# folkol/query-engines

Hardware: AMD Instinct MI355X
Metric: rows/sec filter+project+group-by over 1B-row Arrow batch; % HBM roofline (higher is better)
Workload: dtype int64; 1 GPU; C4: SELECT k, SUM(a+b), COUNT(*), MIN(a), MAX(b) WHERE a > 2^19 GROUP BY k; rows_per_gpu=1000000000, groups=1024, columns=k, a, b int64 (Arrow, no nulls), parallelism=hash-sharded partial aggregate x1

## Files before the change

query-engines_amd/csrc/qe_hashagg.hip:

```cpp
#include <map>
#include <memory>
#include <mutex>

#include "qe_internal.hpp"

namespace qe {

constexpr int HA_THREADS = 512;

__device__ __forceinline__ qi64* lds_keys(char* smem) { return (qi64*)smem; }

__device__ __forceinline__ void lds_init(const Plan& P, char* smem) {
  const int SS = (1 << P.lds_log2) + 2;
  qi64* keys = lds_keys(smem);
  qu32* cst = (qu32*)(smem + P.off_cstar);
  for (int s = threadIdx.x; s < SS; s += blockDim.x) {
    keys[s] = EMPTY_KEY;
    cst[s] = 0;
  }
#pragma unroll
  for (int j = 0; j < QE_MAX_AGGS; ++j) {
    if (j >= P.naggs) break;
    const DAgg& a = P.aggs[j];
    if (a.acc != ACC_NONE) {
      qi64* acc = (qi64*)(smem + P.off_acc[j]);
      const qi64 id = acc_identity(a.acc);
      for (int s = threadIdx.x; s < SS; s += blockDim.x) acc[s] = id;
    }
    if (a.track_nn) {
      qu32* nn = (qu32*)(smem + P.off_nn[j]);
      for (int s = threadIdx.x; s < SS; s += blockDim.x) nn[s] = 0;
    }
    if (acc_has_idx(a.acc)) {
      qu64* ix = (qu64*)(smem + P.off_idx[j]);
      const qu64 id = idx_identity(a.acc);
      for (int s = threadIdx.x; s < 4 * SS; s += blockDim.x) ix[s] = id;
    }
  }
}

__device__ __forceinline__ int lds_find(const Plan& P, char* smem, qi64 key, bool knull) {
  const int S = 1 << P.lds_log2;
  if (knull) return S;
  if (key == EMPTY_KEY) return S + 1;
  return lds_probe(lds_keys(smem), P.lds_log2, key, lds_hash((qu64)key) >> (32 - P.lds_log2));
}

__device__ __forceinline__ void lds_accum_value(const Plan& P, char* smem, int j, int s, qi64 x, qu64 row) {
  const DAgg& a = P.aggs[j];
  qi64* acc = (qi64*)(smem + P.off_acc[j]);
  switch (a.acc) {
    case ACC_SUM_I: atomicAdd((unsigned long long*)&acc[s], (unsigned long long)x); break;
// ... 816 lines not shown
    }
  }
}

__global__ void k_nn_materialize(DTable t, qi32 mask) {
  const qu64 SS = t.cap + 2;
  for (qu64 s = blockIdx.x * (qu64)blockDim.x + threadIdx.x; s < SS; s += (qu64)gridDim.x * blockDim.x)
    for (int j = 0; j < QE_MAX_AGGS; ++j)
      if ((mask >> j) & 1) t.nn[j][s] = t.cstar[s];
}

__device__ __forceinline__ bool gslot_occupied(const DTable& t, qu64 s) {
  return s < t.cap ? t.keys[s] != EMPTY_KEY : t.cstar[s] > 0;
}

__device__ __forceinline__ void wg_newg_begin(qu32* newg) {
  if (threadIdx.x == 0) *newg = 0;
  __syncthreads();
}
__device__ __forceinline__ void wg_newg_end(qu32* newg, qu64* ctl) {
  __syncthreads();
  if (threadIdx.x == 0 && *newg) atomicAdd((unsigned long long*)&ctl[0], (unsigned long long)*newg);
}

__global__ void k_rehash(DTable src, DTable dst, AggMeta m) {
  __shared__ qu32 newg;
  wg_newg_begin(&newg);
  const qu64 SS = src.cap + 2;
  for (qu64 s = blockIdx.x * (qu64)blockDim.x + threadIdx.x; s < SS; s += (qu64)gridDim.x * blockDim.x) {
    if (!gslot_occupied(src, s)) continue;
    const bool knull = s == src.cap;
    const qi64 key = knull ? 0 : (s == src.cap + 1 ? EMPTY_KEY : src.keys[s]);
    qu64 d;
    if (!gtable_find_wg(dst, key, knull, d, &newg)) {
      atomicAdd((unsigned long long*)&dst.ctl[3], 1ull);
      continue;
    }
    gadd_cstar(dst, d, src.cstar[s]);
    for (int j = 0; j < m.naggs; ++j) {
      DAgg a{};
      a.fn = m.fn[j];
      a.acc = m.acc[j];
      qu64 i[4] = {~0ull, ~0ull, ~0ull, ~0ull};
      if (acc_has_idx(a.acc))
        for (int k = 0; k < 4; ++k) i[k] = src.idx[j][k * SS + s];
      gcombine(dst, a.acc, j, d, src.acc[j][s], slot_nn(src, m, j, s), i[0], i[1], i[2], i[3]);
      if (a.acc == ACC_SUM_X && (i[3] & FX_EXT))
        fxe_add_words<true>(dst.ext[j] + d * FXE_WORDS, 0, src.ext[j] + s * FXE_WORDS, FXE_WORDS);
    }
  }
  wg_newg_end(&newg, dst.ctl);
}

__device__ void import_record(const qu8* __restrict__ rec, DTable& dst, const AggMeta& m, qu32* newg) {
  const qi64 key = ((const qi64*)rec)[0];
  const bool knull = ((const qu64*)rec)[1] & 1;
  const qu64 c = ((const qu64*)rec)[2];
  qu64 d;
  if (!gtable_find_wg(dst, key, knull, d, newg)) {
    atomicAdd((unsigned long long*)&dst.ctl[3], 1ull);
    return;
  }
  gadd_cstar(dst, d, c);
  int off = 24;
  for (int j = 0; j < m.naggs; ++j) {
    DAgg a{};
    a.fn = m.fn[j];
    a.acc = m.acc[j];
    const qu64* f = (const qu64*)(rec + off);
    if (a.fn != QE_AGG_COUNT_STAR) {
      if (acc_has_idx(a.acc)) gcombine(dst, a.acc, j, d, (qi64)f[0], f[1], f[2], f[3], f[4], f[5]);
      else gcombine(dst, a.acc, j, d, (qi64)f[0], f[1], ~0ull, ~0ull, ~0ull, ~0ull);
    }
    off += agg_rec_bytes(a.acc);
  }
}

__global__ void k_import(const qu8* __restrict__ recs, qi64 nrec, qi32 rec_bytes, DTable dst, AggMeta m) {
  __shared__ qu32 newg;
  wg_newg_begin(&newg);
  for (qi64 r = blockIdx.x * (qi64)blockDim.x + threadIdx.x; r < nrec; r += (qi64)gridDim.x * blockDim.x)
    import_record(recs + r * rec_bytes, dst, m, &newg);
  wg_newg_end(&newg, dst.ctl);
}

__global__ void k_import_slots(const qu8* __restrict__ slots, qi32 nslots, qi64 slot_records, qi32 rec_bytes,
                               DTable dst, AggMeta m) {
  __shared__ qu32 newg;
  __shared__ qi32 s_ok;
  const qu64 slot_bytes = QE_SLOT_HEADER + (qu64)slot_records * rec_bytes;
  if (threadIdx.x < 64) {
    qu64 mx = 0, tot = 0;
    for (int i = threadIdx.x; i < nslots; i += 64) {
      const qu64* hd = (const qu64*)(slots + (qu64)i * slot_bytes);
      mx = hd[1] > mx ? hd[1] : mx;
      tot += hd[0] < (qu64)slot_records ? hd[0] : (qu64)slot_records;
    }
    for (int off = 32; off > 0; off >>= 1) {
      const qu64 o = __shfl_xor(mx, off);
      mx = o > mx ? o : mx;
      tot += __shfl_xor(tot, off);
    }
    if (threadIdx.x == 0) {
      s_ok = mx <= (qu64)slot_records;
      if (blockIdx.x == 0) {
        dst.ctl[4] = mx;
        dst.ctl[5] = tot;
      }
    }
  }
  wg_newg_begin(&newg);
  if (s_ok) {
    const qi64 total = (qi64)nslots * slot_records;
    for (qi64 r = blockIdx.x * (qi64)blockDim.x + threadIdx.x; r < total; r += (qi64)gridDim.x * blockDim.x) {
      const qi64 sl = r / slot_records, i = r - sl * slot_records;
      const qu8* base = slots + (qu64)sl * slot_bytes;
      if ((qu64)i >= ((const qu64*)base)[0]) continue;
      import_record(base + QE_SLOT_HEADER + (qu64)i * rec_bytes, dst, m, &newg);
    }
  }
  wg_newg_end(&newg, dst.ctl);
// ... 100 lines not shown
    const bool has = s < SS && gslot_occupied(t, s);
    const bool knull = s == t.cap;
    const qi64 key = !has ? 0 : knull ? 0 : (s == t.cap + 1 ? EMPTY_KEY : t.keys[s]);
    const qu32 p = has ? partition_of(key, knull, nparts) : 0;
    const qu64 pos = wave_cursor(cursor, has, p);
    if (has) write_record(dst + pos * (qu64)rec_bytes, t, m, s, key, knull);
    if (m.any_x) {
      const bool ext = has && slot_has_ext(t, m, s);
      const qu64 pe = wave_cursor(cursor, ext, p, FXE_CHUNKS);
      if (ext)
        for (int c = 0; c < FXE_CHUNKS; ++c) write_chunk_record(dst + (pe + c) * (qu64)rec_bytes, t, m, s, key, knull, c);
    }
  }
}

__global__ void k_export_slots(DTable t, AggMeta m, qi32 nparts, qi32 rec_bytes, qi64 slot_records,
                               unsigned long long* cursor, qu8* __restrict__ dst) {
  const qu64 SS = t.cap + 2;
  const qu64 slot_bytes = QE_SLOT_HEADER + (qu64)slot_records * rec_bytes;
  const qu64 stride = (qu64)gridDim.x * blockDim.x;
  for (qu64 s0 = blockIdx.x * (qu64)blockDim.x; s0 < SS; s0 += stride) {
    const qu64 s = s0 + threadIdx.x;
    const bool has = s < SS && gslot_occupied(t, s);
    const bool knull = s == t.cap;
    const qi64 key = !has ? 0 : knull ? 0 : (s == t.cap + 1 ? EMPTY_KEY : t.keys[s]);
    const qu32 p = has ? partition_of(key, knull, nparts) : 0;
    const qu64 pos = wave_cursor(cursor, has, p);
    qu8* base = dst + p * slot_bytes + QE_SLOT_HEADER;
    if (has && pos < (qu64)slot_records) write_record(base + pos * (qu64)rec_bytes, t, m, s, key, knull);
    if (m.any_x) {
      const bool ext = has && slot_has_ext(t, m, s);
      const qu64 pe = wave_cursor(cursor, ext, p, FXE_CHUNKS);
      if (ext)
        for (int c = 0; c < FXE_CHUNKS; ++c)
          if (pe + c < (qu64)slot_records) write_chunk_record(base + (pe + c) * (qu64)rec_bytes, t, m, s, key, knull, c);
    }
  }
}

__global__ void k_slot_headers(const unsigned long long* __restrict__ cursor, qi32 nparts, qu64 slot_bytes,
                               qu8* __restrict__ dst, const qu64* __restrict__ guard) {
  qu64 mx = 0;
  for (int p = threadIdx.x; p < nparts; p += blockDim.x) mx = cursor[p] > mx ? cursor[p] : mx;
  for (int off = 32; off > 0; off >>= 1) {
    const qu64 o = __shfl_xor(mx, off);
    mx = o > mx ? o : mx;
  }
  if (guard && (guard[1] | guard[2] | guard[3])) mx = 1ull << 62;
  for (int p = threadIdx.x; p < nparts; p += blockDim.x) {
    qu64* hd = (qu64*)(dst + (qu64)p * slot_bytes);
    hd[0] = cursor[p];
    hd[1] = mx;
    for (int w = 2; w < QE_SLOT_HEADER / 8; ++w) hd[w] = 0;
  }
}

__global__ void k_occ_count(DTable t, qi64* __restrict__ tile_counts, qi32 tile_slots) {
  __shared__ qi64 part[4];
  const qu64 SS = t.cap + 2;
  const qu64 s0 = (qu64)blockIdx.x * tile_slots;
  qi64 c = 0;
  for (int i = threadIdx.x; i < tile_slots; i += blockDim.x) {
    const qu64 s = s0 + i;
    if (s < SS && gslot_occupied(t, s)) ++c;
  }
  for (int off = 32; off > 0; off >>= 1) c += __shfl_xor(c, off);
  if ((threadIdx.x & 63) == 0) part[threadIdx.x >> 6] = c;
  __syncthreads();
  if (threadIdx.x == 0) tile_counts[blockIdx.x] = part[0] + part[1] + part[2] + part[3];
}

struct OutCols {
  qe_column keys[QE_MAX_KEYS];
  qe_column aggs[QE_MAX_AGGS];
};

__device__ __forceinline__ void set_bit(qu8* bm, qi64 i, bool v) {
  if (v) atomicOr((qu32*)bm + (i >> 5), 1u << (i & 31));
}

__device__ __forceinline__ void store_typed(void* p, qi32 type, qi64 i, qi64 x) {
  switch (type) {
    case QE_TYPE_INT64:
    case QE_TYPE_FLOAT64: ((qi64*)p)[i] = x; break;
    case QE_TYPE_INT32:
    case QE_TYPE_DATE32: ((qi32*)p)[i] = (qi32)x; break;
    default: ((qu8*)p)[i] = (qu8)x;
  }
}

constexpr int FS_WORDS = 512;
__device__ __forceinline__ void put_bit(qu8* gbm, qu32* lbits, int col, qi64 o, bool v) {
  if (!v) return;
  if (lbits) atomicOr(lbits + col * FS_WORDS + (o >> 5), 1u << (o & 31));
  else set_bit(gbm, o, true);
}

__device__ __forceinline__ double fx_sum(const DTable& t, int j, qu64 s, qi64 acc) {
  const qu64 SS = t.cap + 2;
  const qu64* ix = t.idx[j];
  return fx_result((qu64)acc, ix[s], ix[SS + s], ix[2 * SS + s], ix[3 * SS + s], t.ext[j] + s * FXE_WORDS);
}

__device__ __forceinline__ void finalize_slot(const DTable& t, const AggMeta& m, const KeyMeta& km,
                                              const OutCols& out, qu64 s, qi64 o, qu32* lbits = nullptr) {
  const qu64 SS = t.cap + 2;
// ... 25 lines not shown
      case QE_AGG_AVG:
        if (m.acc[j] == ACC_SUM_X)
          val = f64_bits(fx_sum(t, j, s, acc) / (double)nn);
        else
          val = f64_bits(bits_f64(acc) / (double)nn);
        break;
      default:
        if (m.acc[j] == ACC_SUM_X) {
          val = f64_bits(fx_sum(t, j, s, acc));
        } else if (acc_is_f64mm(m.acc[j])) {
          const qu64 i0 = t.idx[j][s], i1 = t.idx[j][SS + s];
          const qu64 i2 = t.idx[j][2 * SS + s], i3 = t.idx[j][3 * SS + s];
          if (i1 != ~0ull && i1 == i0) {
            val = 0x7FF8000000000000ll;
          } else {
            const double d = okey_f64(acc);
            val = d == 0.0 ? f64_bits(i2 < i3 ? -0.0 : 0.0) : f64_bits(d);
          }
        } else {
          val = acc;
        }
    }
    ((qi64*)out.aggs[j].values)[o] = valid ? val : 0;
    if (out.aggs[j].validity) put_bit(out.aggs[j].validity, lbits, QE_MAX_KEYS + j, o, valid);
  }
}

__global__ void k_finalize(DTable t, AggMeta m, KeyMeta km, const qi64* __restrict__ tile_offsets,
                           qi32 tile_slots, OutCols out) {
  __shared__ int wtot[4];
  const qu64 SS = t.cap + 2;
  const int lane = threadIdx.x & 63, wid = threadIdx.x >> 6;
  const qu64 lt = lane ? (~0ull >> (64 - lane)) : 0ull;
  qi64 base = tile_offsets[blockIdx.x];
  for (int it = 0; it < tile_slots; it += blockDim.x) {
    const qu64 s = (qu64)blockIdx.x * tile_slots + it + threadIdx.x;
    const bool occ = (it + (int)threadIdx.x) < tile_slots && s < SS && gslot_occupied(t, s);
    const qu64 b = __ballot(occ);
    if (lane == 0) wtot[wid] = __popcll(b);
    __syncthreads();
    int woff = 0, btot = 0;
    for (int w = 0; w < 4; ++w) {
      woff += w < wid ? wtot[w] : 0;
      btot += wtot[w];
    }
    if (occ) finalize_slot(t, m, km, out, s, base + woff + __popcll(b & lt));
    base += btot;
    __syncthreads();
  }
}

constexpr int FS_THREADS = 1024, FS_PER = 16, FS_WAVES = FS_THREADS / 64;
static_assert(FS_THREADS * FS_PER / 2 / 32 <= FS_WORDS, "LDS bitmaps hold every group of a small table");
__global__ void __launch_bounds__(FS_THREADS) k_finalize_small(DTable t, AggMeta m, KeyMeta km, OutCols out,
                                                               qi64 groups) {
  __shared__ qi32 wcnt[FS_PER][FS_WAVES];
  __shared__ qu64 wbal[FS_PER][FS_WAVES];
  __shared__ qu32 lbits[(QE_MAX_KEYS + QE_MAX_AGGS) * FS_WORDS];
  const qu64 SS = t.cap + 2;
  const int tid = threadIdx.x, lane = tid & 63, wid = tid >> 6;
  const qu64 lt = lane ? (~0ull >> (64 - lane)) : 0ull;
  const int words = (int)((groups + 31) >> 5);
  for (int w = tid; w < (QE_MAX_KEYS + QE_MAX_AGGS) * FS_WORDS; w += FS_THREADS) lbits[w] = 0;
  qu32 occ = 0;
#pragma unroll
  for (int i = 0; i < FS_PER; ++i) {
    const qu64 s = (qu64)i * FS_THREADS + tid;
    if (s < SS && gslot_occupied(t, s)) occ |= 1u << i;
  }
#pragma unroll
  for (int i = 0; i < FS_PER; ++i) {
    const qu64 b = __ballot((occ >> i) & 1);
    if (lane == 0) {
      wbal[i][wid] = b;
      wcnt[i][wid] = __popcll(b);
    }
  }
  __syncthreads();
  static_assert(FS_PER * FS_WAVES == 4 * 64, "four (chunk, wave) counts per lane");
  if (wid == 0) {
    qi32* flat = &wcnt[0][0];
    const qi32 c0 = flat[4 * lane], c1 = flat[4 * lane + 1], c2 = flat[4 * lane + 2], c3 = flat[4 * lane + 3];
    const qi32 sum = c0 + c1 + c2 + c3;
    qi32 inc = sum;
#pragma unroll
    for (int d = 1; d < 64; d <<= 1) {
      const qi32 y = __shfl_up(inc, d);
      if (lane >= d) inc += y;
    }
    const qi32 ex = inc - sum;
    flat[4 * lane] = ex;
    flat[4 * lane + 1] = ex + c0;
    flat[4 * lane + 2] = ex + c0 + c1;
    flat[4 * lane + 3] = ex + c0 + c1 + c2;
  }
  __syncthreads();
  while (occ) {
    const int i = __ffs(occ) - 1;
    occ &= occ - 1;
    const qi64 o = wcnt[i][wid] + __popcll(wbal[i][wid] & lt);
    finalize_slot(t, m, km, out, (qu64)i * FS_THREADS + tid, o, lbits);
  }
  __syncthreads();
  for (int w = tid; w < words; w += FS_THREADS) {
    for (int k = 0; k < QE_MAX_KEYS; ++k)
      if (k < km.nkeys && out.keys[k].validity) ((qu32*)out.keys[k].validity)[w] = lbits[k * FS_WORDS + w];
// ... 5 lines not shown
}

using namespace qe;

struct qe_hashagg {
  qe_ctx* ctx = nullptr;
  int32_t nkeys = 0;
  int32_t key_types[QE_MAX_KEYS] = {};
  int32_t naggs = 0;
  qe_agg_desc aggs[QE_MAX_AGGS] = {};
  int32_t acc[QE_MAX_AGGS] = {};
  KeyMeta km{};
  int32_t rec_bytes = 0;
  int32_t nn_implicit = 0;
  int64_t row_base = 0;
  int64_t known_groups = 0;
  void* table_mem = nullptr;
  DTable t{};
  qu64* ctl = nullptr;
  int32_t lds_log2 = 0;
  int32_t lds_log2_min = 0;
  int64_t expected_groups = 0;
  int64_t create_groups = 0;
  int grid = 0;
  int64_t* part_cnt = nullptr;
  size_t part_cnt_bytes = 0;
  int64_t chunk_cap = 0;
  uint8_t* part_rec = nullptr;
  size_t part_rec_bytes = 0;
  int64_t* part_slc = nullptr;
  size_t part_slc_bytes = 0;
  bool part_wide = false;
  bool narrow_failed = false;
  bool compact_off = false;
  uint8_t* ovf = nullptr;
  uint64_t ovf_cap = 0;
  uint32_t* defer[2] = {nullptr, nullptr};
  size_t defer_words = 0;
  bool defer_dirty[2] = {false, false};
  bool ctl_rows_clean = false;
  hipEvent_t ev[2] = {nullptr, nullptr};
  double last_kernel_ms = 0.0;
  int last_launches = 0;
  int last_specialized = 0;
  uint64_t last_sig = 0;
  std::string jit_note;
  bool async = false;
  bool pending = false;
  std::unique_ptr<qe::Plan> pend_plan;
  size_t pend_lds = 0;
  int pend_out_i = 0;
  uint64_t* ctl_pin = nullptr;
  hipEvent_t ev_ctl = nullptr;
  int poisoned = 0;
  std::string poison_msg;
  qe::Keyed* keyed = nullptr;
  int32_t flags = 0;
  uint64_t version = 0;
};

namespace qe {

int hashagg_expected_groups(const qe_hashagg* h, int64_t* out) {
  QE_CHECK(h && out, QE_ERR_INVALID_ARG, "null argument");
  *out = h->create_groups;
  return QE_OK;
}

qe_ctx* hashagg_ctx(const qe_hashagg* h) { return h ? h->ctx : nullptr; }

HashaggInfo hashagg_info(const qe_hashagg* h) {
  HashaggInfo I{};
  I.ctx = h->ctx;
  I.km = h->km;
  I.rec_bytes = h->rec_bytes;
  I.naggs = h->naggs;
  I.flags = h->flags;
  for (int j = 0; j < h->naggs; ++j) I.aggs[j] = h->aggs[j];
  I.version = h->version;
  I.ctl = (uint64_t*)h->ctl;
  I.keyed = h->keyed;
  return I;
}

static AggMeta agg_meta(const qe_hashagg* h) {
  AggMeta m{};
  m.naggs = h->naggs;
  for (int j = 0; j < h->naggs; ++j) {
    m.fn[j] = h->aggs[j].fn;
    m.acc[j] = h->acc[j];
    m.any_x = m.any_x || h->acc[j] == ACC_SUM_X;
  }
  m.nn_implicit = h->nn_implicit;
  return m;
}

static int32_t all_nn_bits(const qe_hashagg* h) {
  if (!agg_knobs().nn_implicit) return 0;
  int32_t b = 0;
  for (int j = 0; j < h->naggs; ++j)
    if (h->aggs[j].fn != QE_AGG_COUNT_STAR) b |= 1 << j;
  return b;
}

static int nn_materialize(qe_hashagg* h, int32_t mask) {
  mask &= h->nn_implicit;
  if (!mask) return QE_OK;
  const int grid = (int)std::min<uint64_t>(div_up(h->t.cap + 2, 256), 4096);
  hipLaunchKernelGGL(k_nn_materialize, dim3(grid), dim3(256), 0, h->ctx->stream, h->t, (qi32)mask);
  QE_TRY(launch_check("k_nn_materialize"));
  h->nn_implicit &= ~mask;
  return QE_OK;
}

static size_t table_bytes(const qe_hashagg* h, uint64_t cap) {
  const uint64_t SS = cap + 2;
  size_t b = 16 * SS;
  for (int j = 0; j < h->naggs; ++j)
    b += (16 + (acc_has_idx(h->acc[j]) ? 32 : 0) + (h->acc[j] == ACC_SUM_X ? 8 * FXE_WORDS : 0)) * SS;
  return b;
}

static int table_alloc(qe_hashagg* h, uint64_t cap, void** mem, DTable* t, qu64* zero_ctl = nullptr) {
  const size_t bytes = table_bytes(h, cap);
  QE_TRY(dev_alloc(h->ctx, bytes, mem));
  const uint64_t SS = cap + 2;
  char* p = (char*)*mem;
  *t = DTable{};
  t->keys = (qi64*)p;
  p += 8 * SS;
  t->cstar = (qu64*)p;
  p += 8 * SS;
  for (int j = 0; j < h->naggs; ++j) {
    t->acc[j] = (qi64*)p;
    p += 8 * SS;
    t->nn[j] = (qu64*)p;
    p += 8 * SS;
    if (acc_has_idx(h->acc[j])) {
      t->idx[j] = (qu64*)p;
      p += 32 * SS;
    }
  }
  char* e0 = p;
  for (int j = 0; j < h->naggs; ++j)
    if (h->acc[j] == ACC_SUM_X) {
      t->ext[j] = (qu64*)p;
      p += 8 * FXE_WORDS * SS;
    }
  if (p > e0) QE_HIP(hipMemsetAsync(e0, 0, (size_t)(p - e0), h->ctx->stream));
  t->cap = cap;
  t->ctl = h->ctl;
  const int grid = (int)std::min<uint64_t>(div_up(SS, 256), 4096);
  hipLaunchKernelGGL(k_table_init, dim3(grid), dim3(256), 0, h->ctx->stream, *t, agg_meta(h), zero_ctl, 0);
  return launch_check("k_table_init");
}

static int read_ctl(qe_hashagg* h, uint64_t out[8]) {
  void* p;
  QE_TRY(ctx_pinned(h->ctx, 64, &p));
  QE_HIP(hipMemcpyAsync(p, h->ctl, 64, hipMemcpyDeviceToHost, h->ctx->stream));
  QE_TRY(ctx_sync(h->ctx));
  memcpy(out, p, 64);
  QE_CHECK((out[3] & CTL_KEY_TOO_LONG) == 0, QE_ERR_INVALID_ARG,
           "a UTF8 group key is longer than its column's max_len promised (qe_column.max_len)");
  QE_CHECK(out[3] == 0, QE_ERR_CAPACITY, "hash aggregate lost %llu groups (probe limit or overflow area)",
           (unsigned long long)out[3]);
  return QE_OK;
}

static uint64_t next_pow2(uint64_t x) {
  uint64_t p = 1;
  while (p < x) p <<= 1;
  return p;
}

static int table_grow(qe_hashagg* h, uint64_t want_cap) {
  const uint64_t cap = next_pow2(want_cap);
  if (cap <= h->t.cap) return QE_OK;
  void* mem;
  DTable nt;
  QE_TRY(table_alloc(h, cap, &mem, &nt));
  QE_HIP(hipMemsetAsync(h->ctl, 0, 8, h->ctx->stream));
  const int grid = (int)std::min<uint64_t>(div_up(h->t.cap + 2, 256), 8192);
  hipLaunchKernelGGL(k_rehash, dim3(grid), dim3(256), 0, h->ctx->stream, h->t, nt, agg_meta(h));
  QE_TRY(launch_check("k_rehash"));
  uint64_t c[8];
  QE_TRY(read_ctl(h, c));
  QE_CHECK(c[3] == 0, QE_ERR_CAPACITY, "hash table rehash lost %llu groups", (unsigned long long)c[3]);
  dev_free(h->ctx, h->table_mem);
  h->table_mem = mem;
  h->t = nt;
  return QE_OK;
}

static int import_records(qe_hashagg* h, const void* recs, int64_t nrec) {
  if (nrec <= 0) return QE_OK;
  const int grid = (int)std::min<uint64_t>(div_up((uint64_t)nrec, 256), 8192);
  hipLaunchKernelGGL(k_import, dim3(grid), dim3(256), 0, h->ctx->stream, (const uint8_t*)recs, nrec, h->rec_bytes,
                     h->t, agg_meta(h));
  QE_TRY(launch_check("k_import"));
  uint64_t c[8];
  QE_TRY(read_ctl(h, c));
  QE_CHECK(c[3] == 0, QE_ERR_CAPACITY, "hash table import lost %llu groups", (unsigned long long)c[3]);
  return QE_OK;
}

static int ensure_defer(qe_hashagg* h, int64_t n) {
  const size_t words = (size_t)div_up((uint64_t)n, 32);
  if (words <= h->defer_words) return QE_OK;
  for (int i = 0; i < 2; ++i) {
    dev_free(h->ctx, h->defer[i]);
    h->defer[i] = nullptr;
  }
  for (int i = 0; i < 2; ++i) {
    QE_TRY(dev_alloc(h->ctx, words * 4, (void**)&h->defer[i]));
    h->defer_dirty[i] = true;
  }
  h->defer_words = words;
  return QE_OK;
// ... 764 lines not shown
      QE_TRY(settle_pass(h, P, &out_i, &defer_in, &done));
      if (done) break;
    }
  }
  if (pfn && h->narrow_failed) {
    h->narrow_failed = false;
    h->part_wide = true;
    h->chunk_cap = 0;
    P = P_rows;
    pfn = nullptr;
    QE_HIP(hipEventRecord(h->ev[0], ctx->stream));
    continue;
  }
  break;
  }
  if (mp_n)
    h->jit_note = "multi-pass: " + std::to_string(mp_n) + " bucket passes" + (P.lds_compact ? " (compact table)" : "") +
                  (h->last_specialized ? "" : "; " + h->jit_note);
  h->row_base += rows;
  adapt_after_update(h, lds, P.lds_log2);
  return QE_OK;
}

}

extern "C" {

int qe_hashagg_create(qe_ctx* ctx, int32_t nkeys, const int32_t* key_types, int32_t naggs, const qe_agg_desc* aggs,
                      int64_t expected_groups, qe_hashagg** out) {
  return qe_hashagg_create_ex(ctx, nkeys, key_types, naggs, aggs, expected_groups, 0, out);
}

int qe_hashagg_create_ex(qe_ctx* ctx, int32_t nkeys, const int32_t* key_types, int32_t naggs, const qe_agg_desc* aggs,
                         int64_t expected_groups, int32_t flags, qe_hashagg** out) {
  QE_TRY(ctx_enter(ctx));
  QE_CHECK((flags & ~(QE_HASHAGG_DETERMINISTIC | QE_HASHAGG_FAST_FP64)) == 0, QE_ERR_INVALID_ARG, "unknown flags 0x%x",
           flags);
  QE_CHECK((flags & QE_HASHAGG_DETERMINISTIC) == 0 || (flags & QE_HASHAGG_FAST_FP64) == 0, QE_ERR_INVALID_ARG,
           "QE_HASHAGG_DETERMINISTIC and QE_HASHAGG_FAST_FP64 exclude each other");
  const bool det = (flags & QE_HASHAGG_FAST_FP64) == 0;
  QE_CHECK(out, QE_ERR_INVALID_ARG, "null out");
  QE_CHECK(nkeys >= 0 && nkeys <= QE_MAX_KEYS, QE_ERR_UNSUPPORTED, "0..%d group keys supported", QE_MAX_KEYS);
  QE_CHECK(naggs >= 0 && naggs <= QE_MAX_AGGS, QE_ERR_UNSUPPORTED, "0..%d aggregates supported", QE_MAX_AGGS);
  QE_CHECK(nkeys == 0 || key_types, QE_ERR_INVALID_ARG, "null key_types");
  QE_CHECK(naggs == 0 || aggs, QE_ERR_INVALID_ARG, "null aggs");
  qe_hashagg* h = new qe_hashagg();
  h->ctx = ctx;
  h->naggs = naggs;
  h->flags = flags;
  auto bail = [&](int code) {
    for (hipEvent_t e : {h->ev[0], h->ev[1], h->ev_ctl})
      if (e) (void)hipEventDestroy(e);
    if (h->ctl_pin) pinned_slot_free(h->ctl_pin, h->ctx->stream);
    if (h->keyed) keyed_destroy(ctx, h->keyed);
    delete h;
    return code;
  };
  int32_t dev_types[QE_MAX_KEYS] = {};
  {
    int32_t dn = 0;
    const int st = keyed_create(ctx, nkeys, key_types, expected_groups > 0 ? expected_groups : 1024, &h->keyed, &dn,
                                dev_types);
    if (st != QE_OK) return bail(st);
    nkeys = dn;
    key_types = dev_types;
  }
  h->nkeys = nkeys;
  if (nkeys == 0) {
    h->km.mode = 0;
  } else if (nkeys == 1 && (key_types[0] == QE_TYPE_INT64 || key_types[0] == QE_TYPE_FLOAT64)) {
    h->km.mode = 1;
  } else {
    h->km.mode = 2;
    int bit = 0;
    for (int k = 0; k < nkeys; ++k) {
      int w;
      switch (key_types[k]) {
        case QE_TYPE_INT32:
        case QE_TYPE_DATE32: w = 32; break;
        case QE_TYPE_UINT8: w = 8; break;
        default:
          return bail(fail(QE_ERR_UNSUPPORTED,
                           "group key %d: type %d cannot be packed (multi-key groups take uint8/int32/date32)", k,
                           key_types[k]));
      }
      h->km.shift[k] = bit;
      h->km.fmask[k] = (int64_t)((1ull << w) - 1);
      bit += w;
      h->km.nullbit[k] = bit;
      bit += 1;
    }
    if (bit > 63) return bail(fail(QE_ERR_UNSUPPORTED, "group keys need %d bits (max 63)", bit));
  }
  h->km.nkeys = nkeys;
  for (int k = 0; k < nkeys; ++k) {
    h->key_types[k] = key_types[k];
    h->km.type[k] = key_types[k];
  }
  h->rec_bytes = 24;
  for (int j = 0; j < naggs; ++j) {
    const qe_agg_desc& d = aggs[j];
    h->aggs[j] = d;
    const bool f = d.input_type == QE_TYPE_FLOAT64;
    const bool i = d.input_type == QE_TYPE_INT64 || d.input_type == QE_TYPE_INT32 ||
                   d.input_type == QE_TYPE_DATE32 || d.input_type == QE_TYPE_UINT8;
    if (d.fn != QE_AGG_COUNT_STAR && d.fn != QE_AGG_COUNT && !i && !f)
// ... 4 lines not shown
      case QE_AGG_MIN: h->acc[j] = f ? ACC_MIN_F : ACC_MIN_I; break;
      case QE_AGG_MAX: h->acc[j] = f ? ACC_MAX_F : ACC_MAX_I; break;
      case QE_AGG_AVG: h->acc[j] = det ? ACC_SUM_X : ACC_SUM_F; break;
      case QE_AGG_COUNT:
      case QE_AGG_COUNT_STAR: h->acc[j] = ACC_NONE; break;
      default: return bail(fail(QE_ERR_UNSUPPORTED, "aggregate %d: unknown function %d", j, d.fn));
    }
    h->rec_bytes += agg_rec_bytes(h->acc[j]);
  }
  if (hipEventCreate(&h->ev[0]) != hipSuccess || hipEventCreate(&h->ev[1]) != hipSuccess ||
      hipEventCreateWithFlags(&h->ev_ctl, hipEventDisableTiming) != hipSuccess)
    return bail(fail(QE_ERR_DEVICE, "hipEventCreate failed"));
  if (pinned_slot_alloc(&h->ctl_pin) != QE_OK) return bail(QE_ERR_OOM);
  if (dev_alloc(ctx, 64, (void**)&h->ctl) != QE_OK) return bail(fail(QE_ERR_OOM, "control allocation failed"));
  const int64_t eg = expected_groups > 0 ? expected_groups : 1024;
  h->expected_groups = eg;
  h->create_groups = eg;
  const LdsRange lr = lds_table_range(eg, h->acc, naggs, !ctx->jit, lds_budget(ctx));
  h->lds_log2 = lr.log2;
  h->lds_log2_min = lr.log2_min;
  const int per_cu = h->lds_log2 ? std::max<int>(1, std::min<int>(8, (int)((160 * 1024) / lds_bytes_min(h->acc, naggs, h->lds_log2, !ctx->jit)))) : 8;
  h->grid = ctx->num_cus * per_cu;
  if (h->lds_log2) {
    h->ovf_cap = (uint64_t)h->grid * (((uint64_t)1 << h->lds_log2) + 2);
    if (dev_alloc(ctx, h->ovf_cap * h->rec_bytes, (void**)&h->ovf) != QE_OK) {
      dev_free(ctx, h->ctl);
      return bail(fail(QE_ERR_OOM, "overflow area allocation failed"));
    }
  }
  const int st = table_alloc(h, std::max<uint64_t>(1024, next_pow2((uint64_t)(2 * eg))), &h->table_mem, &h->t, h->ctl);
  h->nn_implicit = all_nn_bits(h);
  if (st != QE_OK) {
    dev_free(ctx, h->ovf);
    dev_free(ctx, h->ctl);
    return bail(st);
  }
  h->ctl_rows_clean = true;
  *out = h;
  return QE_OK;
}

int qe_hashagg_destroy(qe_hashagg* h) {
  if (!h) return QE_OK;
  (void)hipSetDevice(h->ctx->device);
  qe_ctx* ctx = h->ctx;
  void* bufs[] = {h->table_mem, h->ctl, h->ovf, h->part_cnt, h->part_rec, h->part_slc, h->defer[0], h->defer[1]};
  for (void* b : bufs) dev_free(ctx, b);
  if (h->keyed) keyed_destroy(ctx, h->keyed);
  for (int i = 0; i < 2; ++i) {
    if (h->ev[i]) (void)hipEventDestroy(h->ev[i]);
  }
  if (h->ev_ctl) (void)hipEventDestroy(h->ev_ctl);
  pinned_slot_free(h->ctl_pin, ctx->stream);
  delete h;
  return QE_OK;
}

int qe_hashagg_last_kernel_kind(qe_hashagg* h, int32_t* specialized, char* note, int32_t note_len) {
  QE_CHECK(h && specialized, QE_ERR_INVALID_ARG, "null argument");
  *specialized = h->last_specialized;
  if (note && note_len > 0) {
    strncpy(note, h->jit_note.c_str(), (size_t)note_len - 1);
    note[note_len - 1] = 0;
  }
  return QE_OK;
}

int qe_hashagg_last_kernel_signature(qe_hashagg* h, uint64_t* sig) {
  QE_CHECK(h && sig, QE_ERR_INVALID_ARG, "null argument");
  *sig = h->last_sig;
  return QE_OK;
}

int qe_hashagg_last_kernel_time(qe_hashagg* h, double* ms, int32_t* launches) {
  QE_CHECK(h && ms, QE_ERR_INVALID_ARG, "null argument");
  QE_TRY(ctx_enter(h->ctx));
  QE_TRY(settle_pending(h));
  *ms = h->last_kernel_ms;
  if (launches) *launches = h->last_launches;
  return QE_OK;
}

int qe_hashagg_last_chunk_stats(qe_hashagg* h, int64_t* chunks, int64_t* full_chunks, int64_t* records) {
  QE_CHECK(h && chunks && full_chunks && records, QE_ERR_INVALID_ARG, "null argument");
  QE_TRY(ctx_enter(h->ctx));
  QE_TRY(settle_pending(h));
  *chunks = *full_chunks = *records = 0;
  if (h->chunk_cap <= 0 || !h->part_cnt) return QE_OK;
  QE_TRY(ctx_sync(h->ctx));
  int64_t ids = 0;
  QE_HIP(hipMemcpy(&ids, h->part_cnt, 8, hipMemcpyDeviceToHost));
  ids = std::max<int64_t>(0, std::min<int64_t>(ids, h->chunk_cap));
  std::vector<int64_t> meta((size_t)ids);
  if (ids) QE_HIP(hipMemcpy(meta.data(), h->part_cnt + 1, (size_t)ids * 8, hipMemcpyDeviceToHost));
  for (const int64_t w : meta) {
    if (w < 0) continue;
    const int64_t fill = w & 0xFFFFFFFFll;
    *chunks += 1;
    *full_chunks += fill == PART_CH ? 1 : 0;
    *records += fill;
  }
  return QE_OK;
}

int qe_hashagg_set_async(qe_hashagg* h, int32_t enable) {
  QE_CHECK(h, QE_ERR_INVALID_ARG, "null state");
// ... 228 lines not shown
  qe_ctx* ctx = h->ctx;
  void* s;
  QE_TRY(ctx_scratch(ctx, (size_t)nparts * 8, &s));
  QE_HIP(hipMemsetAsync(s, 0, (size_t)nparts * 8, ctx->stream));
  const int grid = (int)std::min<uint64_t>(div_up(h->t.cap + 2, 256), 8192);
  hipLaunchKernelGGL(k_export_count, dim3(grid), dim3(256), 0, ctx->stream, h->t, agg_meta(h), nparts,
                     (unsigned long long*)s);
  QE_TRY(launch_check("k_export_count"));
  QE_HIP(hipMemcpyAsync(counts, s, (size_t)nparts * 8, hipMemcpyDeviceToHost, ctx->stream));
  QE_TRY(ctx_sync(ctx));
  return QE_OK;
}

extern "C" {

int qe_hashagg_export(qe_hashagg* h, int32_t nparts, void* dst) {
  QE_CHECK(h && nparts >= 1, QE_ERR_INVALID_ARG, "bad arguments");
  QE_TRY(refuse_dict_records(h));
  QE_TRY(ctx_enter(h->ctx));
  return hashagg_export_raw(h, nparts, dst);
}

}

int qe::hashagg_export_raw(qe_hashagg* h, int32_t nparts, void* dst) {
  qe_ctx* ctx = h->ctx;
  int64_t groups;
  QE_TRY(qe_hashagg_num_groups(h, &groups));
  if (groups == 0) return QE_OK;
  QE_CHECK(dst, QE_ERR_INVALID_ARG, "null destination");
  void* s;
  QE_TRY(ctx_scratch(ctx, (size_t)nparts * 8, &s));
  QE_HIP(hipMemsetAsync(s, 0, (size_t)nparts * 8, ctx->stream));
  const int grid = (int)std::min<uint64_t>(div_up(h->t.cap + 2, 256), 8192);
  hipLaunchKernelGGL(k_export_count, dim3(grid), dim3(256), 0, ctx->stream, h->t, agg_meta(h), nparts,
                     (unsigned long long*)s);
  QE_TRY(launch_check("k_export_count"));
  hipLaunchKernelGGL(k_counts_to_cursors, dim3(1), dim3(64), 0, ctx->stream, (unsigned long long*)s, nparts);
  QE_TRY(launch_check("k_counts_to_cursors"));
  hipLaunchKernelGGL(k_export, dim3(grid), dim3(256), 0, ctx->stream, h->t, agg_meta(h), nparts, h->rec_bytes,
                     (unsigned long long*)s, (uint8_t*)dst);
  QE_TRY(launch_check("k_export"));
  return QE_OK;
}

extern "C" {

int qe_hashagg_export_slots(qe_hashagg* h, int32_t nparts, int64_t slot_records, void* dst) {
  QE_CHECK(h && nparts >= 1 && slot_records >= 1 && dst, QE_ERR_INVALID_ARG, "bad arguments");
  QE_TRY(refuse_dict_records(h));
  QE_TRY(ctx_enter(h->ctx));
  const bool speculative = h->pending;
  qe_ctx* ctx = h->ctx;
  void* s;
  QE_TRY(ctx_scratch(ctx, (size_t)nparts * 8, &s));
  QE_HIP(hipMemsetAsync(s, 0, (size_t)nparts * 8, ctx->stream));
  const int grid = (int)std::min<uint64_t>(div_up(h->t.cap + 2, 256), 8192);
  hipLaunchKernelGGL(k_export_slots, dim3(grid), dim3(256), 0, ctx->stream, h->t, agg_meta(h), nparts, h->rec_bytes,
                     (qi64)slot_records, (unsigned long long*)s, (uint8_t*)dst);
  QE_TRY(launch_check("k_export_slots"));
  const uint64_t slot_bytes = QE_SLOT_HEADER + (uint64_t)slot_records * h->rec_bytes;
  hipLaunchKernelGGL(k_slot_headers, dim3(1), dim3(64), 0, ctx->stream, (const unsigned long long*)s, nparts,
                     (qu64)slot_bytes, (uint8_t*)dst, speculative ? (const qu64*)h->ctl : (const qu64*)nullptr);
  QE_TRY(launch_check("k_slot_headers"));
  return QE_OK;
}

int qe_hashagg_import_slots(qe_hashagg* h, const void* slots, int32_t nslots, int64_t slot_records,
                            int64_t* max_count, int64_t* nrecords) {
  QE_CHECK(h && slots && nslots >= 1 && slot_records >= 1 && max_count, QE_ERR_INVALID_ARG, "bad arguments");
  QE_TRY(refuse_dict_records(h));
  QE_TRY(ctx_enter(h->ctx));
  QE_TRY(settle_pending(h));
  ++h->version;
  QE_TRY(nn_materialize(h, h->nn_implicit));
  qe_ctx* ctx = h->ctx;
  uint64_t groups_before;
  if (h->known_groups >= 0) {
    groups_before = (uint64_t)h->known_groups;
  } else {
    uint64_t c[8];
    QE_TRY(read_ctl(h, c));
    groups_before = c[0];
  }
  const uint64_t bound = groups_before + (uint64_t)nslots * (uint64_t)slot_records;
  if (2 * bound > h->t.cap) QE_TRY(table_grow(h, 2 * bound));
  h->known_groups = -1;
  const int grid = (int)std::min<uint64_t>(div_up((uint64_t)nslots * slot_records, 256), 8192);
  hipLaunchKernelGGL(k_import_slots, dim3(grid), dim3(256), 0, ctx->stream, (const uint8_t*)slots, nslots,
                     (qi64)slot_records, h->rec_bytes, h->t, agg_meta(h));
  QE_TRY(launch_check("k_import_slots"));
  uint64_t c[8];
  QE_TRY(read_ctl(h, c));
  *max_count = (int64_t)c[4];
  if (nrecords) *nrecords = (int64_t)c[5];
  h->known_groups = (int64_t)c[0];
  return QE_OK;
}

int qe_hashagg_import(qe_hashagg* h, const void* records, int64_t nrecords) {
  QE_CHECK(h && nrecords >= 0 && (records || nrecords == 0), QE_ERR_INVALID_ARG, "bad arguments");
  QE_TRY(refuse_dict_records(h));
  QE_TRY(ctx_enter(h->ctx));
  return hashagg_import_raw(h, records, nrecords);
}

int qe_hashagg_key_layout(qe_hashagg* h, int32_t* dictionary_keyed, int32_t* device_nkeys, int32_t* device_types) {
  QE_CHECK(h, QE_ERR_INVALID_ARG, "null state");
  if (dictionary_keyed) *dictionary_keyed = !keyed_dict(h->keyed) ? 0 : keyed_tuple(h->keyed) ? 2 : 1;
  if (device_nkeys) *device_nkeys = h->nkeys;
  if (device_types)
    for (int k = 0; k < QE_MAX_KEYS; ++k) device_types[k] = k < h->nkeys ? h->key_types[k] : 0;
  return QE_OK;
}

}

int qe::hashagg_import_raw(qe_hashagg* h, const void* records, int64_t nrecords) {
  QE_TRY(settle_pending(h));
  if (nrecords == 0) return QE_OK;
  ++h->version;
  QE_TRY(nn_materialize(h, h->nn_implicit));
  h->known_groups = -1;
  uint64_t c[8];
  QE_TRY(read_ctl(h, c));
  if (2 * (c[0] + (uint64_t)nrecords) > h->t.cap) QE_TRY(table_grow(h, 2 * (c[0] + (uint64_t)nrecords)));
  return import_records(h, records, nrecords);
}
```

Measured before the change: 278.7 billion rows/s.

## Add single-workgroup export/import slot kernels with pinned-memory counter publishing

For small hash tables, export and import of partial-aggregate slots now run as one workgroup kernel each. Export keeps its per-partition cursors in LDS and writes the slot headers itself, so it no longer needs the scratch memset, the count kernel or the separate header kernel. Import publishes its group and record counters to pinned host memory, which the host spin-polls instead of doing a blocking control readback. nn_materialize is skipped when the table is known to be empty. This targets launch and synchronisation latency in the merge phase, at the cost of using a single workgroup and burning host CPU while polling.

```diff
diff --git a/query-engines_amd/csrc/qe_hashagg.hip b/query-engines_amd/csrc/qe_hashagg.hip
--- a/query-engines_amd/csrc/qe_hashagg.hip
+++ b/query-engines_amd/csrc/qe_hashagg.hip
@@ -1,3 +1,5 @@
+#include <atomic>
+#include <chrono>
 #include <map>
 #include <memory>
 #include <mutex>
@@ -920,6 +922,7 @@
   wg_newg_end(&newg, dst.ctl);
 }
 
+template <bool ANYX = true>
 __device__ void import_record(const qu8* __restrict__ rec, DTable& dst, const AggMeta& m, qu32* newg) {
   const qi64 key = ((const qi64*)rec)[0];
   const bool knull = ((const qu64*)rec)[1] & 1;
@@ -935,6 +938,7 @@
     DAgg a{};
     a.fn = m.fn[j];
     a.acc = m.acc[j];
+    if (!ANYX) __builtin_assume(a.acc != ACC_SUM_X);
     const qu64* f = (const qu64*)(rec + off);
     if (a.fn != QE_AGG_COUNT_STAR) {
       if (acc_has_idx(a.acc)) gcombine(dst, a.acc, j, d, (qi64)f[0], f[1], f[2], f[3], f[4], f[5]);
@@ -1141,6 +1145,108 @@
     hd[0] = cursor[p];
     hd[1] = mx;
     for (int w = 2; w < QE_SLOT_HEADER / 8; ++w) hd[w] = 0;
+  }
+}
+
+constexpr int XS_THREADS = 1024, XS_MAX_SLOTS = 16384, XS_MAX_PARTS = 1024;
+__global__ void __launch_bounds__(XS_THREADS) k_export_slots_small(DTable t, AggMeta m, qi32 nparts, qi32 rec_bytes,
+                                                                   qi64 slot_records, qu8* __restrict__ dst,
+                                                                   const qu64* __restrict__ guard) {
+  __shared__ unsigned long long cursor[XS_MAX_PARTS];
+  __shared__ qu64 wmx[XS_THREADS / 64];
+  const qu64 SS = t.cap + 2;
+  const qu64 slot_bytes = QE_SLOT_HEADER + (qu64)slot_records * rec_bytes;
+  const int tid = threadIdx.x;
+  for (int p = tid; p < nparts; p += XS_THREADS) cursor[p] = 0;
+  __syncthreads();
+  for (qu64 s0 = 0; s0 < SS; s0 += XS_THREADS) {
+    const qu64 s = s0 + tid;
+    const bool has = s < SS && gslot_occupied(t, s);
+    const bool knull = s == t.cap;
+    const qi64 key = !has ? 0 : knull ? 0 : (s == t.cap + 1 ? EMPTY_KEY : t.keys[s]);
+    const qu32 p = has ? partition_of(key, knull, nparts) : 0;
+    const qu64 pos = wave_cursor(cursor, has, p);
+    qu8* base = dst + p * slot_bytes + QE_SLOT_HEADER;
+    if (has && pos < (qu64)slot_records) write_record(base + pos * (qu64)rec_bytes, t, m, s, key, knull);
+    if (m.any_x) {
+      const bool ext = has && slot_has_ext(t, m, s);
+      const qu64 pe = wave_cursor(cursor, ext, p, FXE_CHUNKS);
+      if (ext)
+        for (int c = 0; c < FXE_CHUNKS; ++c)
+          if (pe + c < (qu64)slot_records) write_chunk_record(base + (pe + c) * (qu64)rec_bytes, t, m, s, key, knull, c);
+    }
+  }
+  __syncthreads();
+  qu64 mx = 0;
+  for (int p = threadIdx.x; p < nparts; p += XS_THREADS) mx = cursor[p] > mx ? cursor[p] : mx;
+  for (int off = 32; off > 0; off >>= 1) {
+    const qu64 o = __shfl_xor(mx, off);
+    mx = o > mx ? o : mx;
+  }
+  if ((threadIdx.x & 63) == 0) wmx[threadIdx.x >> 6] = mx;
+  __syncthreads();
+  for (int w = 0; w < XS_THREADS / 64; ++w) mx = wmx[w] > mx ? wmx[w] : mx;
+  if (guard && (guard[1] | guard[2] | guard[3])) mx = 1ull << 62;
+  constexpr int HW = QE_SLOT_HEADER / 8;
+  for (int i = threadIdx.x; i < nparts * HW; i += XS_THREADS) {
+    const int p = i / HW, w = i - p * HW;
+    ((qu64*)(dst + (qu64)p * slot_bytes))[w] = w == 0 ? (qu64)cursor[p] : w == 1 ? mx : 0;
+  }
+}
+
+template <bool ANYX>
+__global__ void __launch_bounds__(XS_THREADS) k_import_slots_small(const qu8* __restrict__ slots, qi32 nslots,
+                                                                   qi64 slot_records, qi32 rec_bytes, DTable dst,
+                                                                   AggMeta m, qu64* pin, qu64 tag) {
+  __shared__ qu32 newg;
+  __shared__ qi32 s_ok;
+  __shared__ qu64 s_mx, s_tot;
+  const qu64 slot_bytes = QE_SLOT_HEADER + (qu64)slot_records * rec_bytes;
+  const int tid = threadIdx.x;
+  if (threadIdx.x < 64) {
+    qu64 mx = 0, tot = 0;
+    for (int i = threadIdx.x; i < nslots; i += 64) {
+      const qu64* hd = (const qu64*)(slots + (qu64)i * slot_bytes);
+      mx = hd[1] > mx ? hd[1] : mx;
+      tot += hd[0] < (qu64)slot_records ? hd[0] : (qu64)slot_records;
+    }
+    for (int off = 32; off > 0; off >>= 1) {
+      const qu64 o = __shfl_xor(mx, off);
+      mx = o > mx ? o : mx;
+      tot += __shfl_xor(tot, off);
+    }
+    if (threadIdx.x == 0) {
+      s_ok = mx <= (qu64)slot_records;
+      s_mx = mx;
+      s_tot = tot;
+    }
+  }
+  wg_newg_begin(&newg);
+  if (s_ok) {
+    const int total = nslots * (int)slot_records, sr = (int)slot_records;
+    for (int r0 = 0; r0 < total; r0 += XS_THREADS) {
+      const int r = r0 + tid;
+      const qu8* rec = nullptr;
+      if (r < total) {
+        const int sl = r / sr, i = r - sl * sr;
+        const qu8* base = slots + (qu64)sl * slot_bytes;
+        if ((qu64)i < ((const qu64*)base)[0]) rec = base + QE_SLOT_HEADER + (qu64)i * rec_bytes;
+      }
+      if (rec) import_record<ANYX>(rec, dst, m, &newg);
+    }
+  }
+  __threadfence();
+  __syncthreads();
+  if (tid == 0) {
+    const qu64 groups = atomicAdd((unsigned long long*)&dst.ctl[0], (unsigned long long)newg) + newg;
+    const qu64 lost = __hip_atomic_load(&dst.ctl[3], __ATOMIC_RELAXED, __HIP_MEMORY_SCOPE_AGENT);
+    dst.ctl[4] = s_mx;
+    dst.ctl[5] = s_tot;
+    __hip_atomic_store(&pin[0], groups, __ATOMIC_RELAXED, __HIP_MEMORY_SCOPE_SYSTEM);
+    __hip_atomic_store(&pin[1], s_mx, __ATOMIC_RELAXED, __HIP_MEMORY_SCOPE_SYSTEM);
+    __hip_atomic_store(&pin[2], s_tot, __ATOMIC_RELAXED, __HIP_MEMORY_SCOPE_SYSTEM);
+    __hip_atomic_store(&pin[3], lost, __ATOMIC_RELAXED, __HIP_MEMORY_SCOPE_SYSTEM);
+    __hip_atomic_store(&pin[4], tag, __ATOMIC_RELEASE, __HIP_MEMORY_SCOPE_SYSTEM);
   }
 }
 
@@ -1272,6 +1378,7 @@
 
 constexpr int FS_THREADS = 1024, FS_PER = 16, FS_WAVES = FS_THREADS / 64;
 static_assert(FS_THREADS * FS_PER / 2 / 32 <= FS_WORDS, "LDS bitmaps hold every group of a small table");
+static_assert(XS_MAX_SLOTS == FS_THREADS * FS_PER, "one bound for every single-workgroup table walk");
 __global__ void __launch_bounds__(FS_THREADS) k_finalize_small(DTable t, AggMeta m, KeyMeta km, OutCols out,
                                                                qi64 groups) {
   __shared__ qi32 wcnt[FS_PER][FS_WAVES];
@@ -1383,6 +1490,7 @@
   int pend_out_i = 0;
   uint64_t* ctl_pin = nullptr;
   hipEvent_t ev_ctl = nullptr;
+  uint64_t* imp_pin = nullptr;
   int poisoned = 0;
   std::string poison_msg;
   qe::Keyed* keyed = nullptr;
@@ -1437,6 +1545,10 @@
 static int nn_materialize(qe_hashagg* h, int32_t mask) {
   mask &= h->nn_implicit;
   if (!mask) return QE_OK;
+  if (h->known_groups == 0 && !h->pending) {
+    h->nn_implicit &= ~mask;
+    return QE_OK;
+  }
   const int grid = (int)std::min<uint64_t>(div_up(h->t.cap + 2, 256), 4096);
   hipLaunchKernelGGL(k_nn_materialize, dim3(grid), dim3(256), 0, h->ctx->stream, h->t, (qi32)mask);
   QE_TRY(launch_check("k_nn_materialize"));
@@ -1496,6 +1608,46 @@
            "a UTF8 group key is longer than its column's max_len promised (qe_column.max_len)");
   QE_CHECK(out[3] == 0, QE_ERR_CAPACITY, "hash aggregate lost %llu groups (probe limit or overflow area)",
            (unsigned long long)out[3]);
+  return QE_OK;
+}
+
+static int import_slots_small(qe_hashagg* h, const void* slots, int32_t nslots, int64_t slot_records,
+                              int64_t* max_count, int64_t* nrecords) {
+  qe_ctx* ctx = h->ctx;
+  if (!h->imp_pin) QE_TRY(pinned_slot_alloc(&h->imp_pin));
+  volatile uint64_t* pv = h->imp_pin;
+  const uint64_t tag = h->version;
+  pv[4] = 0;
+  const AggMeta m = agg_meta(h);
+  if (m.any_x)
+    hipLaunchKernelGGL(k_import_slots_small<true>, dim3(1), dim3(XS_THREADS), 0, ctx->stream, (const uint8_t*)slots,
+                       nslots, (qi64)slot_records, h->rec_bytes, h->t, m, (qu64*)h->imp_pin, (qu64)tag);
+  else
+    hipLaunchKernelGGL(k_import_slots_small<false>, dim3(1), dim3(XS_THREADS), 0, ctx->stream, (const uint8_t*)slots,
+                       nslots, (qi64)slot_records, h->rec_bytes, h->t, m, (qu64*)h->imp_pin, (qu64)tag);
+  QE_TRY(launch_check("k_import_slots_small"));
+  auto t0 = std::chrono::steady_clock::now();
+  for (uint32_t i = 1; pv[4] != tag; ++i) {
+    if ((i & 1023) != 0) continue;
+    if (std::chrono::steady_clock::now() - t0 < std::chrono::microseconds(50)) continue;
+    t0 = std::chrono::steady_clock::now();
+    const hipError_t e = hipStreamQuery(ctx->stream);
+    if (e == hipSuccess) {
+      QE_CHECK(pv[4] == tag, QE_ERR_DEVICE, "slot import finished without publishing its counters");
+      break;
+    }
+    if (e != hipErrorNotReady) return fail(QE_ERR_DEVICE, "slot import kernel failed: %s", hipGetErrorString(e));
+    (void)hipGetLastError();
+  }
+  std::atomic_thread_fence(std::memory_order_acquire);
+  const uint64_t groups = pv[0], mx = pv[1], tot = pv[2], lost = pv[3];
+  QE_CHECK((lost & CTL_KEY_TOO_LONG) == 0, QE_ERR_INVALID_ARG,
+           "a UTF8 group key is longer than its column's max_len promised (qe_column.max_len)");
+  QE_CHECK(lost == 0, QE_ERR_CAPACITY, "hash aggregate lost %llu groups (probe limit or overflow area)",
+           (unsigned long long)lost);
+  *max_count = (int64_t)mx;
+  if (nrecords) *nrecords = (int64_t)tot;
+  h->known_groups = (int64_t)groups;
   return QE_OK;
 }
 
@@ -2366,6 +2518,7 @@
     for (hipEvent_t e : {h->ev[0], h->ev[1], h->ev_ctl})
       if (e) (void)hipEventDestroy(e);
     if (h->ctl_pin) pinned_slot_free(h->ctl_pin, h->ctx->stream);
+    if (h->imp_pin) pinned_slot_free(h->imp_pin, h->ctx->stream);
     if (h->keyed) keyed_destroy(ctx, h->keyed);
     delete h;
     return code;
@@ -2476,6 +2629,7 @@
   }
   if (h->ev_ctl) (void)hipEventDestroy(h->ev_ctl);
   pinned_slot_free(h->ctl_pin, ctx->stream);
+  pinned_slot_free(h->imp_pin, ctx->stream);
   delete h;
   return QE_OK;
 }
@@ -2810,6 +2964,12 @@
   QE_TRY(ctx_enter(h->ctx));
   const bool speculative = h->pending;
   qe_ctx* ctx = h->ctx;
+  if (h->t.cap + 2 <= (uint64_t)XS_MAX_SLOTS && nparts <= XS_MAX_PARTS) {
+    const qu64* guard = speculative ? (const qu64*)h->ctl : (const qu64*)nullptr;
+    hipLaunchKernelGGL(k_export_slots_small, dim3(1), dim3(XS_THREADS), 0, ctx->stream, h->t, agg_meta(h), nparts,
+                       h->rec_bytes, (qi64)slot_records, (uint8_t*)dst, guard);
+    return launch_check("k_export_slots_small");
+  }
   void* s;
   QE_TRY(ctx_scratch(ctx, (size_t)nparts * 8, &s));
   QE_HIP(hipMemsetAsync(s, 0, (size_t)nparts * 8, ctx->stream));
@@ -2844,6 +3004,8 @@
   const uint64_t bound = groups_before + (uint64_t)nslots * (uint64_t)slot_records;
   if (2 * bound > h->t.cap) QE_TRY(table_grow(h, 2 * bound));
   h->known_groups = -1;
+  if ((uint64_t)nslots * (uint64_t)slot_records <= (uint64_t)XS_MAX_SLOTS)
+    return import_slots_small(h, slots, nslots, slot_records, max_count, nrecords);
   const int grid = (int)std::min<uint64_t>(div_up((uint64_t)nslots * slot_records, 256), 8192);
   hipLaunchKernelGGL(k_import_slots, dim3(grid), dim3(256), 0, ctx->stream, (const uint8_t*)slots, nslots,
                      (qi64)slot_records, h->rec_bytes, h->t, agg_meta(h));
```

Measured after the change: 278.4 billion rows/s. About the same (-0.1%).
